# KirillHit/snn_for_object_detection

Measured on AMD Instinct MI355X. Metric: event-frames/sec (BxT) SODa-3M GEN1 304x240 fwd+bwd, higher is better.
Workload: dtype f32 (16-bit split products)

## Files before the change

### snn_for_object_detection_amd/csrc/conv_halo.hip

```cpp
#include <stdlib.h>
#include <type_traits>
#include "snn_common.h"

namespace {

constexpr int kThreads = 256;
constexpr int HBM_ = 128;
constexpr int HCELLS = 288;
constexpr int HPIECE = HCELLS * 64;
constexpr int NPASS = HCELLS / 32;
static_assert(NPASS == 9, "one halo staging pass per tap");

typedef __bf16 bf16x8 __attribute__((ext_vector_type(8)));
typedef __bf16 bf16x2 __attribute__((ext_vector_type(2)));
typedef _Float16 f16x8 __attribute__((ext_vector_type(8)));
typedef _Float16 f16x2 __attribute__((ext_vector_type(2)));
typedef float f32x2 __attribute__((ext_vector_type(2)));
typedef unsigned u32x2 __attribute__((ext_vector_type(2)));
typedef unsigned u32x4 __attribute__((ext_vector_type(4)));

constexpr float kF16WeightScale = 256.0f;
constexpr float kF16ActScale = 16.0f;
constexpr float kF16Unscale = 1.0f / (kF16WeightScale * kF16ActScale);

struct HaloGeom {
    int64_t ldx, ldy, ld_add, ld_add2;
    int N, H, W, Cin, Cout;
    int PW, PH;
    int G;
    int group_cells;
    int tiles_per_group, tiles, tiles_per_xcd, ntiles_n;
    unsigned magic_pw, magic_ph;
    int out_vec;
    double* bn_partial;
    int OH, OW;
    int tiles_x, tiles_img;
    float x_th;
};

__device__ __forceinline__ unsigned udiv_small(unsigned n, unsigned magic) { return __umulhi(n, magic); }

template <bool F16>
__device__ __forceinline__ void split4(const f32x4& v, u32x2& hi, u32x2& lo) {
#pragma unroll
    for (int e = 0; e < 4; e += 2) {
        if constexpr (F16) {
            const float a = v[e] * kF16ActScale, b = v[e + 1] * kF16ActScale;
            const f16x2 ph = __builtin_convertvector(f32x2{a, b}, f16x2);
            const f16x2 pl = __builtin_convertvector(f32x2{a - (float)ph[0], b - (float)ph[1]}, f16x2);
            hi[e >> 1] = __builtin_bit_cast(unsigned, ph);
            lo[e >> 1] = __builtin_bit_cast(unsigned, pl);
        } else {
            f32x2 rest = {v[e], v[e + 1]};
            const bf16x2 ph = __builtin_convertvector(rest, bf16x2);
            const unsigned bits = __builtin_bit_cast(unsigned, ph);
            rest[0] -= __builtin_bit_cast(float, bits << 16);
            rest[1] -= __builtin_bit_cast(float, bits & 0xffff0000u);
            const bf16x2 pl = __builtin_convertvector(rest, bf16x2);
            hi[e >> 1] = bits;
            lo[e >> 1] = __builtin_bit_cast(unsigned, pl);
        }
    }
}

__device__ __forceinline__ double partner8(double v) {
    const u32x2 u = __builtin_bit_cast(u32x2, v);
    const u32x2 o = {(unsigned)__builtin_amdgcn_update_dpp(0, (int)u[0], 0x128, 0xf, 0xf, false),
                     (unsigned)__builtin_amdgcn_update_dpp(0, (int)u[1], 0x128, 0xf, 0xf, false)};
    return __builtin_bit_cast(double, o);
}
__device__ __forceinline__ double partner16(double v) {
    const u32x2 u = __builtin_bit_cast(u32x2, v);
    const u32x2 o = {__builtin_amdgcn_permlane16_swap(u[0], u[0], false, false)[0],
                     __builtin_amdgcn_permlane16_swap(u[1], u[1], false, false)[0]};
    return __builtin_bit_cast(double, o);
}
__device__ __forceinline__ double partner32(double v) {
    const u32x2 u = __builtin_bit_cast(u32x2, v);
    const u32x2 o = {__builtin_amdgcn_permlane32_swap(u[0], u[0], false, false)[0],
                     __builtin_amdgcn_permlane32_swap(u[1], u[1], false, false)[0]};
    return __builtin_bit_cast(double, o);
}

__device__ __forceinline__ int cell_slot_off(int cell, int slot) { return cell * 64 + ((slot ^ ((cell >> 2) & 3)) << 4); }


constexpr int RTH = 4, RTW = 32, RPITCH = RTW + 2, RCELLS = (RTH + 2) * RPITCH;

template <int CO, bool F16, int ABL = 0, bool RECT = false, bool SBF = false, bool XSP = false>
__global__ __launch_bounds__(kThreads, 2) void k_conv_halo3(const float* __restrict__ x,
                                                           const unsigned char* __restrict__ wimg,
                                                           float* __restrict__ y, HaloGeom g,
                                                           const float* __restrict__ addend,
                                                           const float* __restrict__ addend2) {
    constexpr int WM = CO == 32 ? 4 : 2, WN = 4 / WM, TM = CO == 32 ? 1 : 2, TN = CO == 32 ? 1 : CO / 64;
    static_assert(CO == 32 || CO == 64 || CO == 128, "channel tile");
    constexpr int BTILE = (CO / 32) * 4096;
    constexpr int NDMA = (CO / 32) * 4 / 4;
    constexpr int ES = SBF ? 2 : 4;
    static_assert(!SBF || (!F16 && ABL == 0), "bf16 storage: bf16 MFMA, plain variant");
    static_assert(!XSP || (F16 && !SBF && ABL == 0), "spikes from potentials: the forward arithmetic, plain variant");
    constexpr int HC = RECT ? (RCELLS + 31) / 32 * 32 : HCELLS;
    constexpr int HP = HC * 64;
    constexpr int RED_BYTES = (F16 || SBF) ? 4 * (CO == 128 ? 64 : 32) * 16 : 0;
    __shared__ __attribute__((aligned(16))) unsigned char smem[2 * HP + 2 * BTILE + RED_BYTES];
    unsigned char* Aimg = smem;
    unsigned char* Bimg = smem + 2 * HP;

    const int tid = threadIdx.x, lane = tid & 63;
    const int wave = __builtin_amdgcn_readfirstlane(tid >> 6);
    const int wm = wave / WN, wn = wave % WN;
    const int r = lane & 31, h = lane >> 5;

    const int bq = blockIdx.x >> 3;
    const int tile = (blockIdx.x & 7) * g.tiles_per_xcd + bq / g.ntiles_n;
    if (tile >= g.tiles) return;
    const int n0c = (bq % g.ntiles_n) * CO;
    int grp, kt, c0 = 0, x0 = 0, y0 = 0, n0, nb;
    [[maybe_unused]] int ty = 0, tx = 0;
    if constexpr (RECT) {
        n0 = tile / g.tiles_img;
        const int rem = tile - n0 * g.tiles_img;
        ty = rem / g.tiles_x;
        tx = rem - ty * g.tiles_x;
        grp = n0 / g.G;
        kt = (n0 - grp * g.G) * g.tiles_img + rem;
        nb = n0;
    } else {
        grp = tile / g.tiles_per_group;
        kt = tile - grp * g.tiles_per_group;
        c0 = kt * HBM_;
        const int R0g = c0 / g.PW;
        x0 = c0 - R0g * g.PW;
        const int ng = R0g / g.PH;
        y0 = R0g - ng * g.PH;
        n0 = grp * g.G + ng;
        nb = n0 > 0 ? n0 - 1 : 0;
    }
    const int pitch = RECT ? RPITCH : g.PW;

    const int quad = tid & 7;
    const int64_t ipix = (int64_t)g.H * g.W;
    const int64_t xbytes = ((((int64_t)g.N - nb) * ipix - 1) * g.ldx + g.Cin) * ES;
    __amdgpu_buffer_rsrc_t rs_x = __builtin_amdgcn_make_buffer_rsrc(
        reinterpret_cast<char*>(const_cast<float*>(x)) + (int64_t)nb * ipix * g.ldx * ES, 0,
        xbytes > 0x7fffffffLL ? 0x7fffffff : (int)xbytes, 0x00020000);
    unsigned voff[NPASS];
    int awr[NPASS];
#pragma unroll
    for (int p = 0; p < NPASS; ++p) {
        const int cell = p * 32 + (tid >> 3);
        int xx, yy, n;
        bool ok;
        if constexpr (RECT) {
            const int rr = cell / RPITCH, cc = cell - rr * RPITCH;
            yy = ty * RTH - 1 + rr;
            xx = tx * RTW - 1 + cc;
            n = n0;
            ok = cell < RCELLS && yy >= 0 && yy < g.H && xx >= 0 && xx < g.W;
        } else {
            const unsigned u = (unsigned)(x0 + cell + g.PW - 1);
            const unsigned dR = udiv_small(u, g.magic_pw);
            xx = (int)(u - dR * g.PW);
            const unsigned v = (unsigned)(y0 + (int)dR + g.PH - 2);
            const unsigned dn = udiv_small(v, g.magic_ph);
            yy = (int)(v - dn * g.PH);
            n = n0 - 1 + (int)dn;
            ok = n >= 0 && n < g.N && xx < g.W && yy < g.H;
        }
        const int64_t pix = (int64_t)(n - nb) * ipix + (int64_t)yy * g.W + xx;
        voff[p] = ok ? (unsigned)((pix * g.ldx + quad * 4) * ES) : 0x80000000u;
        awr[p] = cell_slot_off(cell, quad >> 1) + (quad & 1) * 8;
    }

    int cellbase[TM];
#pragma unroll
    for (int i = 0; i < TM; ++i)
        cellbase[i] = RECT ? (wm * TM + i + 1) * RPITCH + 1 + r : g.PW + 1 + (wm * TM + i) * 32 + r;
    const int nchunks = g.Cin >> 5;
    const int co_tiles = g.Cout >> 5;
    const unsigned char* wsrc = wimg + (int64_t)(n0c >> 5) * 4096 + lane * 16;
    const unsigned lds_b = (unsigned)(size_t)(__attribute__((address_space(3))) unsigned char*)Bimg;
    auto dma_b = [&](int kk, int buf) {
        if constexpr (SBF)
            if (wave & 1) return;
        const int chunk = kk / 9, tap = kk - chunk * 9;
        const unsigned char* src = wsrc + ((int64_t)(tap * nchunks + chunk) * co_tiles) * 4096 + wave * 1024;
        const unsigned dst = lds_b + buf * BTILE + wave * 1024;
#pragma unroll
        for (int q = 0; q < NDMA; ++q) {
            unsigned keep;
            asm volatile("s_mov_b32 %0, m0\n\ts_mov_b32 m0, %2\n\ts_nop 0\n\tglobal_load_lds_dwordx4 %1, off\n\ts_mov_b32 m0, %0"
                         : "=&s"(keep)
                         : "v"(src + q * 4096), "s"(__builtin_amdgcn_readfirstlane(dst + q * 4096))
                         : "memory");
        }
    };

    using PReg = typename std::conditional<SBF, u32x2, f32x4>::type;
    PReg pf[NPASS];
    auto store_halo = [&]() {
#pragma unroll
        for (int p = 0; p < NPASS; ++p) {
            if constexpr (RECT)
                if (p * 32 >= HC) continue;
            if constexpr (SBF) {
                *reinterpret_cast<u32x2*>(Aimg + awr[p]) = pf[p];
            } else if constexpr (XSP) {
                const u32x2 hi = {(pf[p][0] > g.x_th ? 0x4C00u : 0u) | (pf[p][1] > g.x_th ? 0x4C000000u : 0u),
                                  (pf[p][2] > g.x_th ? 0x4C00u : 0u) | (pf[p][3] > g.x_th ? 0x4C000000u : 0u)};
                *reinterpret_cast<u32x2*>(Aimg + awr[p]) = hi;
            } else {
                u32x2 hi, lo;
                split4<F16>(pf[p], hi, lo);
                *reinterpret_cast<u32x2*>(Aimg + awr[p]) = hi;
                *reinterpret_cast<u32x2*>(Aimg + HP + awr[p]) = lo;
            }
        }
    };
    auto load_pass = [&](int off) -> PReg {
        if constexpr (SBF) return __builtin_bit_cast(u32x2, __builtin_amdgcn_raw_buffer_load_b64(rs_x, off, 0, 0));
        else return __builtin_bit_cast(f32x4, __builtin_amdgcn_raw_buffer_load_b128(rs_x, off, 0, 0));
    };

    f32x16 acc[TM][TN];
#pragma unroll
    for (int i = 0; i < TM; ++i)
#pragma unroll
        for (int j = 0; j < TN; ++j)
#pragma unroll
            for (int e = 0; e < 16; ++e) acc[i][j][e] = 0.f;

    auto kstep = [&](int tapoff, const unsigned char* Bb) {
#pragma unroll
        for (int ks = 0; ks < 2; ++ks) {
            bf16x8 ah[TM], al[TM], bh[TN], bl[TN];
#pragma unroll
            for (int i = 0; i < TM; ++i) {
                const int off = cell_slot_off(cellbase[i] + tapoff, 2 * ks + h);
                if constexpr (ABL & 16) {
                    if (i == 0 && ks == 0) ah[0] = *reinterpret_cast<const bf16x8*>(Aimg + off);
                    ah[i] = ah[0];
                    al[i] = ah[0];
                    continue;
                }
                ah[i] = *reinterpret_cast<const bf16x8*>(Aimg + off);
                if constexpr (!SBF && !XSP) al[i] = *reinterpret_cast<const bf16x8*>(Aimg + HP + off);
            }
#pragma unroll
            for (int j = 0; j < TN; ++j) {
                const int off = (wn * TN + j) * 4096 + ks * 2048 + lane * 16;
                bh[j] = *reinterpret_cast<const bf16x8*>(Bb + off);
                if constexpr (!SBF) bl[j] = *reinterpret_cast<const bf16x8*>(Bb + off + 1024);
            }
#pragma unroll
            for (int i = 0; i < TM; ++i)
#pragma unroll
                for (int j = 0; j < TN; ++j) {
                    if constexpr (SBF) {
                        acc[i][j] = __builtin_amdgcn_mfma_f32_32x32x16_bf16(ah[i], bh[j], acc[i][j], 0, 0, 0);
                    } else if constexpr (XSP) {
                        const f16x8 xah = __builtin_bit_cast(f16x8, ah[i]);
                        const f16x8 xbh = __builtin_bit_cast(f16x8, bh[j]), xbl = __builtin_bit_cast(f16x8, bl[j]);
                        acc[i][j] = __builtin_amdgcn_mfma_f32_32x32x16_f16(xah, xbl, acc[i][j], 0, 0, 0);
                        acc[i][j] = __builtin_amdgcn_mfma_f32_32x32x16_f16(xah, xbh, acc[i][j], 0, 0, 0);
                    } else if constexpr (F16) {
                        const f16x8 xah = __builtin_bit_cast(f16x8, ah[i]), xal = __builtin_bit_cast(f16x8, al[i]);
                        const f16x8 xbh = __builtin_bit_cast(f16x8, bh[j]), xbl = __builtin_bit_cast(f16x8, bl[j]);
                        acc[i][j] = __builtin_amdgcn_mfma_f32_32x32x16_f16(xal, xbh, acc[i][j], 0, 0, 0);
                        acc[i][j] = __builtin_amdgcn_mfma_f32_32x32x16_f16(xah, xbl, acc[i][j], 0, 0, 0);
                        acc[i][j] = __builtin_amdgcn_mfma_f32_32x32x16_f16(xah, xbh, acc[i][j], 0, 0, 0);
                    } else {
                        acc[i][j] = __builtin_amdgcn_mfma_f32_32x32x16_bf16(al[i], bh[j], acc[i][j], 0, 0, 0);
                        acc[i][j] = __builtin_amdgcn_mfma_f32_32x32x16_bf16(ah[i], bl[j], acc[i][j], 0, 0, 0);
                        acc[i][j] = __builtin_amdgcn_mfma_f32_32x32x16_bf16(ah[i], bh[j], acc[i][j], 0, 0, 0);
                    }
                }
        }
    };

    dma_b(0, 0);
#pragma unroll
    for (int p = 0; p < NPASS; ++p) pf[p] = load_pass((int)voff[p]);
    store_halo();
    asm volatile("s_waitcnt vmcnt(0) lgkmcnt(0)\n\ts_barrier" ::: "memory");

    const int nk = nchunks * 9;
#pragma unroll 1
    for (int chunk = 0; chunk < nchunks; ++chunk) {
        const bool more = chunk + 1 < nchunks;
        const int cbytes = (chunk + 1) * 32 * ES;
#pragma unroll
        for (int tap = 0; tap < 9; ++tap) {
            const int kk = chunk * 9 + tap;
            const int cur = kk & 1;
            if constexpr (!(ABL & 1))
                if (kk + 1 < nk) dma_b(kk + 1, cur ^ 1);
            __builtin_amdgcn_sched_barrier(0);
            if constexpr (!(ABL & 4)) {
                if (more) pf[tap] = load_pass((int)(voff[tap] + (unsigned)cbytes));
            }
            __builtin_amdgcn_sched_barrier(0);
            const int kh = tap / 3, kw = tap - 3 * kh;
            kstep((kh - 1) * pitch + (kw - 1), Bimg + cur * BTILE);
            if constexpr (ABL & 2) asm volatile("" ::: "memory");
            else if constexpr (ABL & 4) asm volatile("s_waitcnt vmcnt(0) lgkmcnt(0)\n\ts_barrier" ::: "memory");
            else asm volatile("s_waitcnt vmcnt(0) lgkmcnt(0)\n\ts_barrier" ::: "memory");
        }
        if (more) {
            store_halo();
            asm volatile("s_waitcnt lgkmcnt(0)\n\ts_barrier" ::: "memory");
        }
    }

    constexpr int EW = TN * 32 + 4;
    constexpr int LPR = TN * 8;
    constexpr int RPP = 64 / LPR;
    float* stage = reinterpret_cast<float*>(smem) + wave * 32 * EW;
    const bool ovec = g.out_vec != 0;
    const int lrow = lane / LPR, c4 = (lane % LPR) * 4;
    const int nch = n0c + wn * TN * 32 + c4;
    const int cells_left = g.group_cells - c0;
    double ssum[4] = {0.0, 0.0, 0.0, 0.0}, qsum[4] = {0.0, 0.0, 0.0, 0.0};
    const bool stats = (F16 || SBF) && g.bn_partial != nullptr;
    auto cell_pixel = [&](int m, int64_t& pix) -> bool {
        int xx, yy, n;
        bool ok;
        if constexpr (RECT) {
            yy = ty * RTH + (m >> 5);
            xx = tx * RTW + (m & 31);
            n = n0;
            ok = yy < g.H && xx < g.W && nch < g.Cout;
        } else {
            const unsigned u = (unsigned)(x0 + m);
            const unsigned dR = udiv_small(u, g.magic_pw);
            xx = (int)(u - dR * g.PW);
            const unsigned v = (unsigned)(y0 + (int)dR);
            const unsigned dn = udiv_small(v, g.magic_ph);
            yy = (int)(v - dn * g.PH);
            n = n0 + (int)dn;
            ok = m < cells_left && xx < g.W && yy < g.H && n < g.N && nch < g.Cout;
        }
        pix = ((int64_t)n * g.H + yy) * g.W + xx;
        return ok;
    };
    typedef SnnStore<SBF> St;
    constexpr int NPS = 32 / RPP;
    const bool prefetch_add = ovec && (addend != nullptr || addend2 != nullptr) && !(ABL & 8);
#pragma unroll
    for (int i = 0; i < TM; ++i) {
        f32x4 pa1[NPS], pa2[NPS];
        int64_t ppix[NPS];
        unsigned okmask = 0;
        if (prefetch_add) {
#pragma unroll
            for (int pass = 0; pass < NPS; ++pass) {
                const bool ok = cell_pixel((wm * TM + i) * 32 + pass * RPP + lrow, ppix[pass]);
                okmask |= ok ? 1u << pass : 0u;
                const int64_t pc = ok ? ppix[pass] : 0;
                const int nc = ok ? nch : 0;
                const f32x4 zero = {0.f, 0.f, 0.f, 0.f};
                pa1[pass] = addend ? St::ld4_last(addend, pc * g.ld_add + nc) : zero;
                pa2[pass] = addend2 ? St::ld4_last(addend2, pc * g.ld_add2 + nc) : zero;
            }
        }
#pragma unroll
        for (int j = 0; j < TN; ++j)
#pragma unroll
            for (int e = 0; e < 16; ++e)
                stage[((e & 3) + 8 * (e >> 2) + 4 * h) * EW + j * 32 + r] = F16 ? acc[i][j][e] * kF16Unscale : acc[i][j][e];
        asm volatile("s_waitcnt lgkmcnt(0)" ::: "memory");
        if (prefetch_add) {
#pragma unroll
            for (int pass = 0; pass < NPS; ++pass) {
                f32x4 val = *reinterpret_cast<const f32x4*>(&stage[(pass * RPP + lrow) * EW + c4]);
                if (addend) val += pa1[pass];
                if (addend2) val += pa2[pass];
                if ((okmask >> pass) & 1u) St::st4(y, ppix[pass] * g.ldy + nch, val);
            }
            asm volatile("s_waitcnt lgkmcnt(0)" ::: "memory");
            continue;
        }
#pragma unroll
        for (int pass = 0; pass < NPS; ++pass) {
            const int row = pass * RPP + lrow;
            int64_t pix;
            const bool ok = cell_pixel((wm * TM + i) * 32 + row, pix);
            f32x4 val = *reinterpret_cast<const f32x4*>(&stage[row * EW + c4]);
            if (!ok) continue;
            if constexpr (ABL & 8) {
                asm volatile("" :: "v"(val[0]), "v"(val[1]), "v"(val[2]), "v"(val[3]));
                continue;
            }
            if (ovec) {
                if (addend) val += St::ld4_last(addend, pix * g.ld_add + nch);
                if (addend2) val += St::ld4_last(addend2, pix * g.ld_add2 + nch);
                St::st4(y, pix * g.ldy + nch, val);
            } else {
#pragma unroll
                for (int q = 0; q < 4; ++q) {
                    float o = val[q];
                    if (addend) o += St::ld1(addend, pix * g.ld_add + nch + q);
                    if (addend2) o += St::ld1(addend2, pix * g.ld_add2 + nch + q);
                    St::st1(y, pix * g.ldy + nch + q, o);
                }
            }
            if (stats) {
#pragma unroll
                for (int q = 0; q < 4; ++q) {
                    const double d = (double)val[q];
                    ssum[q] += d;
                    qsum[q] = fma(d, d, qsum[q]);
                }
            }
        }
        asm volatile("s_waitcnt lgkmcnt(0)" ::: "memory");
    }
    if (stats) {
#pragma unroll
        for (int q = 0; q < 4; ++q) {
            if constexpr (LPR <= 8) {
                ssum[q] += partner8(ssum[q]);
                qsum[q] += partner8(qsum[q]);
            }
            ssum[q] += partner16(ssum[q]);
            qsum[q] += partner16(qsum[q]);
            ssum[q] += partner32(ssum[q]);
            qsum[q] += partner32(qsum[q]);
        }
        double* red = reinterpret_cast<double*>(smem + 2 * HP + 2 * BTILE);
        if (lane >= 48 && lane < 48 + LPR) {
#pragma unroll
            for (int q = 0; q < 4; ++q) {
                red[((wave * LPR + lane - 48) * 4 + q) * 2 + 0] = ssum[q];
                red[((wave * LPR + lane - 48) * 4 + q) * 2 + 1] = qsum[q];
            }
        }
        __syncthreads();
        if (tid < CO) {
            const int wn_ = tid / (TN * 32), cc = tid % (TN * 32);
            double s = 0.0, q2 = 0.0;
#pragma unroll
            for (int wm_ = 0; wm_ < WM; ++wm_) {
                const double* src = red + (((wm_ * WN + wn_) * LPR * 4) + cc) * 2;
                s += src[0];
                q2 += src[1];
            }
            if (n0c + tid < g.Cout) {
                double* dstp = g.bn_partial + snn_bn_partial_index(grp, kt, n0c + tid, g.tiles_per_group, g.Cout);
                dstp[0] = s;
                dstp[1] = q2;
            }
        }
    }
}

constexpr int SPITCH = RTW + 1, SCELLS = (RTH + 1) * SPITCH;
template <bool SBF = false, bool RECT = false>
__global__ __launch_bounds__(kThreads, 2) void k_conv_s2dgrad3(const float* __restrict__ x,
                                                              const unsigned char* __restrict__ wimg,
                                                              float* __restrict__ y,
                                                              HaloGeom g, const float* __restrict__ addend,
                                                              const float* __restrict__ addend2) {
    constexpr int CO = 64, TN = 2;
    constexpr int ES = SBF ? 2 : 4;
    constexpr int BTILE = (CO / 32) * 4096;
    constexpr int NDMA = (CO / 32) * 4 / 4;
    __shared__ __attribute__((aligned(16))) unsigned char smem[2 * HPIECE + 2 * BTILE];
    unsigned char* Aimg = smem;
    unsigned char* Bimg = smem + 2 * HPIECE;

    const int tid = threadIdx.x, lane = tid & 63;
    const int wave = __builtin_amdgcn_readfirstlane(tid >> 6);
    const int r = lane & 31, h = lane >> 5;

    const int bq = blockIdx.x >> 3;
    const int tile = (blockIdx.x & 7) * g.tiles_per_xcd + bq / g.ntiles_n;
    if (tile >= g.tiles) return;
    const int n0c = (bq % g.ntiles_n) * CO;
    int c0 = 0, x0 = 0, y0 = 0, n0;
    [[maybe_unused]] int ty = 0, tx = 0;
    if constexpr (RECT) {
        n0 = tile / g.tiles_img;
        const int rem = tile - n0 * g.tiles_img;
        ty = rem / g.tiles_x;
        tx = rem - ty * g.tiles_x;
    } else {
        c0 = tile * HBM_;
        const int R0g = c0 / g.PW;
        x0 = c0 - R0g * g.PW;
        n0 = R0g / g.PH;
        y0 = R0g - n0 * g.PH;
    }
    const int nb = n0;
    const int pitch = RECT ? SPITCH : g.PW;

    const int quad = tid & 7;
    const int64_t ipix = (int64_t)g.H * g.W;
    const int64_t xbytes = ((((int64_t)g.N - nb) * ipix - 1) * g.ldx + g.Cin) * ES;
    __amdgpu_buffer_rsrc_t rs_x = __builtin_amdgcn_make_buffer_rsrc(
        reinterpret_cast<char*>(const_cast<float*>(x)) + (int64_t)nb * ipix * g.ldx * ES, 0,
        xbytes > 0x7fffffffLL ? 0x7fffffff : (int)xbytes, 0x00020000);
    unsigned voff[NPASS];
    int awr[NPASS];
#pragma unroll
    for (int p = 0; p < NPASS; ++p) {
        const int cell = p * 32 + (tid >> 3);
        int xx, yy, n;
        bool ok;
        if constexpr (RECT) {
            const int rr = cell / SPITCH, cc = cell - rr * SPITCH;
            yy = ty * RTH + rr;
            xx = tx * RTW + cc;
            n = n0;
            ok = cell < SCELLS && xx < g.W && yy < g.H;
        } else {
            const unsigned u = (unsigned)(x0 + cell);
            const unsigned dR = udiv_small(u, g.magic_pw);
            xx = (int)(u - dR * g.PW);
            const unsigned v = (unsigned)(y0 + (int)dR);
            const unsigned dn = udiv_small(v, g.magic_ph);
            yy = (int)(v - dn * g.PH);
            n = n0 + (int)dn;
            ok = n < g.N && xx < g.W && yy < g.H;
        }
        const int64_t pix = (int64_t)(n - nb) * ipix + (int64_t)yy * g.W + xx;
        voff[p] = ok ? (unsigned)((pix * g.ldx + quad * 4) * ES) : 0x80000000u;
        awr[p] = cell_slot_off(cell, quad >> 1) + (quad & 1) * 8;
    }
    const int cellbase = RECT ? wave * SPITCH + r : wave * 32 + r;
    const int nchunks = g.Cin >> 5;
    const int co_tiles = g.Cout >> 5;
    const unsigned char* wsrc = wimg + (int64_t)(n0c >> 5) * 4096 + lane * 16;
    const unsigned lds_b = (unsigned)(size_t)(__attribute__((address_space(3))) unsigned char*)Bimg;
    auto dma_b = [&](int kk, int buf) {
        if constexpr (SBF)
            if (wave & 1) return;
        const int chunk = kk / 9, tap = kk - chunk * 9;
        const unsigned char* src = wsrc + ((int64_t)((8 - tap) * nchunks + chunk) * co_tiles) * 4096 + wave * 1024;
        const unsigned dst = lds_b + buf * BTILE + wave * 1024;
#pragma unroll
        for (int q = 0; q < NDMA; ++q) {
            unsigned keep;
            asm volatile("s_mov_b32 %0, m0\n\ts_mov_b32 m0, %2\n\ts_nop 0\n\tglobal_load_lds_dwordx4 %1, off\n\ts_mov_b32 m0, %0"
                         : "=&s"(keep)
                         : "v"(src + q * 4096), "s"(__builtin_amdgcn_readfirstlane(dst + q * 4096))
                         : "memory");
        }
    };
    using PReg = typename std::conditional<SBF, u32x2, f32x4>::type;
    PReg pf[NPASS];
    auto store_halo = [&]() {
#pragma unroll
        for (int p = 0; p < NPASS; ++p) {
            if constexpr (SBF) {
                *reinterpret_cast<u32x2*>(Aimg + awr[p]) = pf[p];
            } else {
                u32x2 hi, lo;
                split4<false>(pf[p], hi, lo);
                *reinterpret_cast<u32x2*>(Aimg + awr[p]) = hi;
                *reinterpret_cast<u32x2*>(Aimg + HPIECE + awr[p]) = lo;
            }
        }
    };
    auto load_pass = [&](int off) -> PReg {
        if constexpr (SBF) return __builtin_bit_cast(u32x2, __builtin_amdgcn_raw_buffer_load_b64(rs_x, off, 0, 0));
        else return __builtin_bit_cast(f32x4, __builtin_amdgcn_raw_buffer_load_b128(rs_x, off, 0, 0));
    };
    f32x16 acc[4][TN];
#pragma unroll
    for (int c = 0; c < 4; ++c)
#pragma unroll
        for (int j = 0; j < TN; ++j)
#pragma unroll
            for (int e = 0; e < 16; ++e) acc[c][j][e] = 0.f;

    auto kstep = [&](int tapoff, const unsigned char* Bb, f32x16 (&a)[TN]) {
#pragma unroll
        for (int ks = 0; ks < 2; ++ks) {
            const int off = cell_slot_off(cellbase + tapoff, 2 * ks + h);
            const bf16x8 ah = *reinterpret_cast<const bf16x8*>(Aimg + off);
            bf16x8 al = ah;
            if constexpr (!SBF) al = *reinterpret_cast<const bf16x8*>(Aimg + HPIECE + off);
#pragma unroll
            for (int j = 0; j < TN; ++j) {
                const int boff = j * 4096 + ks * 2048 + lane * 16;
                const bf16x8 bh = *reinterpret_cast<const bf16x8*>(Bb + boff);
                if constexpr (!SBF) {
                    const bf16x8 bl = *reinterpret_cast<const bf16x8*>(Bb + boff + 1024);
                    a[j] = __builtin_amdgcn_mfma_f32_32x32x16_bf16(al, bh, a[j], 0, 0, 0);
                    a[j] = __builtin_amdgcn_mfma_f32_32x32x16_bf16(ah, bl, a[j], 0, 0, 0);
                }
                a[j] = __builtin_amdgcn_mfma_f32_32x32x16_bf16(ah, bh, a[j], 0, 0, 0);
            }
        }
    };

    dma_b(0, 0);
#pragma unroll
    for (int p = 0; p < NPASS; ++p) pf[p] = load_pass((int)voff[p]);
    store_halo();
    asm volatile("s_waitcnt vmcnt(0) lgkmcnt(0)\n\ts_barrier" ::: "memory");

    const int nk = nchunks * 9;
#pragma unroll 1
    for (int chunk = 0; chunk < nchunks; ++chunk) {
        const bool more = chunk + 1 < nchunks;
        const int cbytes = (chunk + 1) * 32 * ES;
#pragma unroll
        for (int tap = 0; tap < 9; ++tap) {
            const int kk = chunk * 9 + tap;
            const int cur = kk & 1;
            if (kk + 1 < nk) dma_b(kk + 1, cur ^ 1);
            __builtin_amdgcn_sched_barrier(0);
            if (more) pf[tap] = load_pass((int)(voff[tap] + (unsigned)cbytes));
            __builtin_amdgcn_sched_barrier(0);
            const int kh = tap / 3, kw = tap - 3 * kh;
            const int ph = kh == 1 ? 0 : 1, pw = kw == 1 ? 0 : 1;
            const int dh = kh == 0 ? 1 : 0, dw = kw == 0 ? 1 : 0;
            kstep(dh * pitch + dw, Bimg + cur * BTILE, acc[2 * ph + pw]);
            asm volatile("s_waitcnt vmcnt(0) lgkmcnt(0)\n\ts_barrier" ::: "memory");
        }
        if (more) {
            store_halo();
            asm volatile("s_waitcnt lgkmcnt(0)\n\ts_barrier" ::: "memory");
        }
    }

    constexpr int EW = TN * 32 + 4, LPR = TN * 8, RPP = 64 / LPR;
    float* stage = reinterpret_cast<float*>(smem) + wave * 32 * EW;
    const bool ovec = g.out_vec != 0;
    const int lrow = lane / LPR, c4 = (lane % LPR) * 4;
    const int nch = n0c + c4;
    const int cells_left = g.group_cells - c0;
#pragma unroll
    for (int cls = 0; cls < 4; ++cls) {
        const int ph = cls >> 1, pw = cls & 1;
#pragma unroll
        for (int j = 0; j < TN; ++j)
#pragma unroll
            for (int e = 0; e < 16; ++e)
                stage[((e & 3) + 8 * (e >> 2) + 4 * h) * EW + j * 32 + r] = acc[cls][j][e];
        asm volatile("s_waitcnt lgkmcnt(0)" ::: "memory");
#pragma unroll
        for (int pass = 0; pass < 32 / RPP; ++pass) {
            const int row = pass * RPP + lrow;
            const int m = wave * 32 + row;
            int aa, bb, n;
            bool inside;
            if constexpr (RECT) {
                aa = ty * RTH + wave;
                bb = tx * RTW + row;
                n = n0;
                inside = true;
            } else {
                const unsigned u = (unsigned)(x0 + m);
                const unsigned dR = udiv_small(u, g.magic_pw);
                bb = (int)(u - dR * g.PW);
                const unsigned v = (unsigned)(y0 + (int)dR);
                const unsigned dn = udiv_small(v, g.magic_ph);
                aa = (int)(v - dn * g.PH);
                n = n0 + (int)dn;
                inside = m < cells_left && n < g.N;
            }
            const int hi = 2 * aa + ph, wi = 2 * bb + pw;
            const bool ok = inside && bb < g.W && aa < g.H && hi < g.OH && wi < g.OW && nch < g.Cout;
            f32x4 val = *reinterpret_cast<const f32x4*>(&stage[row * EW + c4]);
            if (!ok) continue;
            const int64_t pix = ((int64_t)n * g.OH + hi) * g.OW + wi;
            typedef SnnStore<SBF> St;
            if (ovec) {
                if (addend) val += St::ld4_last(addend, pix * g.ld_add + nch);
                if (addend2) val += St::ld4_last(addend2, pix * g.ld_add2 + nch);
                St::st4(y, pix * g.ldy + nch, val);
            } else {
#pragma unroll
                for (int q = 0; q < 4; ++q) {
                    float o = val[q];
                    if (addend) o += St::ld1(addend, pix * g.ld_add + nch + q);
                    if (addend2) o += St::ld1(addend2, pix * g.ld_add2 + nch + q);
                    St::st1(y, pix * g.ldy + nch + q, o);
                }
            }
        }
        asm volatile("s_waitcnt lgkmcnt(0)" ::: "memory");
    }
}

template <bool F16>
__global__ void k_weight_frag_image(const float* __restrict__ flat_src, unsigned char* __restrict__ flat_dst,
                                    const int64_t* __restrict__ table, int flip) {
    const int64_t* row = table + (int64_t)blockIdx.y * 4;
    const float* src = flat_src + row[0];
    unsigned char* dst = flat_dst + row[1];
    const int O = (int)row[2], I = (int)row[3];
    const int ot_n = O >> 5, ic_n = I >> 5;
    const int64_t total = (int64_t)9 * ic_n * ot_n * 2 * 64;
    for (int64_t idx = (int64_t)blockIdx.x * blockDim.x + threadIdx.x; idx < total; idx += (int64_t)gridDim.x * blockDim.x) {
        const int lane = (int)(idx & 63);
        const int ks = (int)((idx >> 6) & 1);
        int64_t rest = idx >> 7;
        const int ot = (int)(rest % ot_n); rest /= ot_n;
        const int ic = (int)(rest % ic_n);
        const int tap = (int)(rest / ic_n);
        const int r = lane & 31, h = lane >> 5;
        const int st = flip ? 8 - tap : tap;
        const float* p = src + ((int64_t)(ot * 32 + r) * 9 + st) * I + ic * 32 + ks * 16 + h * 8;
        const f32x4 v0 = *reinterpret_cast<const f32x4*>(p), v1 = *reinterpret_cast<const f32x4*>(p + 4);
        u32x4 hi, lo;
#pragma unroll
        for (int e = 0; e < 8; e += 2) {
            const float a0 = e < 4 ? v0[e] : v1[e - 4], a1 = e < 4 ? v0[e + 1] : v1[e - 3];
            if (F16) {
                const float a = a0 * kF16WeightScale, b = a1 * kF16WeightScale;
                const f16x2 ph = __builtin_convertvector(f32x2{a, b}, f16x2);
                const f16x2 pl = __builtin_convertvector(f32x2{a - (float)ph[0], b - (float)ph[1]}, f16x2);
                hi[e >> 1] = __builtin_bit_cast(unsigned, ph);
                lo[e >> 1] = __builtin_bit_cast(unsigned, pl);
            } else {
                f32x2 rr = {a0, a1};
                const bf16x2 ph = __builtin_convertvector(rr, bf16x2);
                const unsigned bits = __builtin_bit_cast(unsigned, ph);
                rr[0] -= __builtin_bit_cast(float, bits << 16);
                rr[1] -= __builtin_bit_cast(float, bits & 0xffff0000u);
                const bf16x2 pl = __builtin_convertvector(rr, bf16x2);
                hi[e >> 1] = bits;
                lo[e >> 1] = __builtin_bit_cast(unsigned, pl);
            }
        }
        unsigned char* o = dst + ((((int64_t)(tap * ic_n + ic) * ot_n + ot) * 2 + ks) * 2) * 1024 + lane * 16;
        *reinterpret_cast<u32x4*>(o) = hi;
        *reinterpret_cast<u32x4*>(o + 1024) = lo;
    }
}

static int halo_mode(int64_t N, int H, int W, int Cin, int Cout) {
    if (N <= 0 || H <= 0 || W <= 0) return 0;
    if (Cin % 32 != 0 || Cin < 32 || (Cout % 64 != 0 && Cout != 32)) return 0;
    if (W + 1 <= 79) {
        if (N * (int64_t)(H + 1) * (W + 1) >= 0x7fffffffLL) return 0;
        return 1;
    }
    const int64_t tiles = N * snn_ceil_div(H, RTH) * snn_ceil_div(W, RTW);
    return tiles < 0x7fffffffLL ? 2 : 0;
}
static bool halo_shape_ok(int64_t N, int H, int W, int Cin, int Cout) { return halo_mode(N, H, W, Cin, Cout) != 0; }

static bool s2dgrad_rect(int Wo) { return 128 + (Wo + 1) + 2 > HCELLS; }
static bool s2dgrad_shape_ok(int64_t N, int H, int W, int Cin, int Ho, int Wo, int Cout) {
    if (N <= 0 || H <= 0 || W <= 0) return false;
    if (Ho != (H - 1) / 2 + 1 || Wo != (W - 1) / 2 + 1) return false;
    if (Cout % 32 != 0 || Cout < 32 || Cin % 64 != 0) return false;
    if (s2dgrad_rect(Wo)) return N * snn_ceil_div(Ho, RTH) * snn_ceil_div(Wo, RTW) < 0x7fffffffLL;
    if (N * (int64_t)(Ho + 1) * (Wo + 1) >= 0x7fffffffLL) return false;
    return true;
}

struct HaloPlan {
    int mode;
    int co_tile, ntiles_n;
    int G;
    int tiles_x, tiles_img;
    int group_cells;
    int tiles_per_group, tiles, tiles_per_xcd, grid;
};
static void plan_grid(HaloPlan& p) {
    if (p.tiles * (int64_t)p.ntiles_n + 8 >= 0x7fffffffLL) {
        p.mode = 0;
        return;
    }
    p.tiles_per_xcd = (int)snn_ceil_div(p.tiles, 8);
    const int64_t grid = (int64_t)p.tiles_per_xcd * 8 * p.ntiles_n;
    if (grid > 0x7fffffffLL) p.mode = 0;
    p.grid = (int)grid;
}
static HaloPlan halo_plan(int64_t N, int H, int W, int Cin, int Cout, int G) {
    HaloPlan p = {};
    p.mode = halo_mode(N, H, W, Cin, Cout);
    if (p.mode == 0 || G <= 0 || N % G != 0) return HaloPlan{};
    p.G = G;
    p.co_tile = Cout % 128 == 0 ? 128 : (Cout % 64 == 0 ? 64 : 32);
    p.ntiles_n = Cout / p.co_tile;
    p.tiles_x = (int)snn_ceil_div(W, RTW);
    p.tiles_img = p.tiles_x * (int)snn_ceil_div(H, RTH);
    int64_t tiles;
    if (p.mode == 2) {
        p.tiles_per_group = G * p.tiles_img;
        tiles = N * (int64_t)p.tiles_img;
    } else {
        const int64_t group_cells = (int64_t)G * (H + 1) * (W + 1);
        p.group_cells = (int)group_cells;
        p.tiles_per_group = (int)snn_ceil_div(group_cells, HBM_);
        tiles = (N / G) * p.tiles_per_group;
    }
    if (tiles >= 0x7fffffffLL) return HaloPlan{};
    p.tiles = (int)tiles;
    plan_grid(p);
    return p;
}
static HaloPlan s2dgrad_plan(int64_t N, int H, int W, int Cin, int Ho, int Wo, int Cout) {
    HaloPlan p = {};
    if (!s2dgrad_shape_ok(N, H, W, Cin, Ho, Wo, Cout)) return p;
    p.mode = s2dgrad_rect(Wo) ? 2 : 1;
    p.G = (int)N;
    p.co_tile = 64;
    p.ntiles_n = Cin / 64;
    p.tiles_x = (int)snn_ceil_div(Wo, RTW);
    p.tiles_img = p.tiles_x * (int)snn_ceil_div(Ho, RTH);
    if (p.mode == 2) {
        p.tiles_per_group = p.tiles_img;
        p.tiles = (int)(N * p.tiles_img);
    } else {
        const int64_t cells = N * (int64_t)(Ho + 1) * (Wo + 1);
        p.group_cells = (int)cells;
        p.tiles_per_group = (int)snn_ceil_div(cells, HBM_);
        p.tiles = p.tiles_per_group;
    }
    plan_grid(p);
    return p;
}
static int plan_out(const HaloPlan& p, int* out) {
    const int v[7] = {p.mode, p.co_tile, p.tiles, p.tiles_per_group, p.tiles_per_xcd, p.ntiles_n, p.grid};
    for (int i = 0; i < 7; ++i) out[i] = v[i];
    return p.mode == 0 ? 1 : 0;
}

static HaloGeom halo_geom(const HaloPlan& hp, int64_t N, int H, int W, int Cin, int64_t ld_in, int OH, int OW, int Cout,
                          const void* out, int64_t ld_out, const void* addend, int64_t ld_add, const void* addend2,
                          int64_t ld_add2, bool bf16, double* bn_partial, float x_th) {
    HaloGeom g = {};
    g.ldx = ld_in; g.ldy = ld_out; g.ld_add = ld_add; g.ld_add2 = ld_add2;
    g.N = (int)N; g.H = H; g.W = W; g.Cin = Cin; g.Cout = Cout;
    g.OH = OH; g.OW = OW;
    g.PW = W + 1; g.PH = H + 1;
    g.G = hp.G;
    g.tiles_x = hp.tiles_x;
    g.tiles_img = hp.tiles_img;
    g.group_cells = hp.group_cells;
    g.tiles_per_group = hp.tiles_per_group;
    g.tiles = hp.tiles;
    g.ntiles_n = hp.ntiles_n;
    g.tiles_per_xcd = hp.tiles_per_xcd;
    g.magic_pw = magic_u32(g.PW); g.magic_ph = magic_u32(g.PH);
    g.out_vec = multiples(4, {ld_out, addend ? ld_add : 0, addend2 ? ld_add2 : 0}) && aligned(bf16 ? 8 : 16, {out, addend, addend2});
    g.bn_partial = bn_partial;
    g.x_th = x_th;
    return g;
}
}

extern "C" int snn_conv3x3_s2_dgrad_supported(int64_t N, int H, int W, int Cin, int Ho, int Wo, int Cout) {
    return s2dgrad_shape_ok(N, H, W, Cin, Ho, Wo, Cout) ? 1 : 0;
}

extern "C" int snn_conv3x3_s2_dgrad(const float* dy, int64_t lddy, const void* wt_image, float* dx, int64_t lddx, int64_t N,
                                    int H, int W, int Cin, int Ho, int Wo, int Cout, const float* addend, int64_t ld_addend,
                                    const float* addend2, int64_t ld_addend2, int precision, void* stream) {
    SNN_REQUIRE(dy && wt_image && dx, "snn_conv3x3_s2_dgrad: null pointer");
    SNN_REQUIRE(precision == SNN_PREC_BF16X3 || precision == SNN_PREC_BF16S,
                "snn_conv3x3_s2_dgrad: precision must be SNN_PREC_BF16X3 or SNN_PREC_BF16S (got %d)", precision);
    const bool sbf = precision == SNN_PREC_BF16S;
    SNN_REQUIRE(s2dgrad_shape_ok(N, H, W, Cin, Ho, Wo, Cout),
                "snn_conv3x3_s2_dgrad: shape not covered (N %lld, %dx%d -> %dx%d, %d -> %d channels; ask "
                "snn_conv3x3_s2_dgrad_supported)", (long long)N, H, W, Ho, Wo, Cin, Cout);
    SNN_REQUIRE(lddy >= Cout && lddx >= Cin && lddy % 4 == 0, "snn_conv3x3_s2_dgrad: bad pixel strides (%lld, %lld)",
                (long long)lddy, (long long)lddx);
    SNN_REQUIRE(aligned(sbf ? 8 : 16, {dy}) && aligned(16, {wt_image}),
                "snn_conv3x3_s2_dgrad: dy (16 bytes; 8 for bf16) and the weight image (16) must be aligned");
    SNN_REQUIRE(!addend || ld_addend >= Cin, "snn_conv3x3_s2_dgrad: addend pixel stride smaller than channel count");
    SNN_REQUIRE(!addend2 || ld_addend2 >= Cin, "snn_conv3x3_s2_dgrad: addend2 pixel stride smaller than channel count");
    const HaloPlan hp = s2dgrad_plan(N, H, W, Cin, Ho, Wo, Cout);
    SNN_REQUIRE(hp.mode != 0, "snn_conv3x3_s2_dgrad: grid too large");
    const bool rect = hp.mode == 2;
    if (rect)
        SNN_REQUIRE((int64_t)Ho * Wo * lddy * 4 < 0x7fffffffLL, "snn_conv3x3_s2_dgrad: a dy image must span less than 2 GiB");
    else
        SNN_REQUIRE((int64_t)4 * Ho * Wo * lddy * 4 < 0x7fffffffLL, "snn_conv3x3_s2_dgrad: four dy images must span less than 2 GiB");
    const HaloGeom g = halo_geom(hp, N, Ho, Wo, Cout, lddy, H, W, Cin, dx, lddx, addend, ld_addend, addend2, ld_addend2, sbf,
                                 nullptr, 0.0f);
    dispatch(
        [&](auto SBF, auto RECT) {
            hipLaunchKernelGGL((k_conv_s2dgrad3<SBF(), RECT()>), dim3((unsigned)hp.grid), dim3(kThreads), 0, (hipStream_t)stream,
                               dy, static_cast<const unsigned char*>(wt_image), dx, g, addend, addend2);
            return true;
        },
        Flag{sbf}, Flag{rect});
    SNN_CHECK_LAUNCH("snn_conv3x3_s2_dgrad");
    return 0;
}

extern "C" int snn_conv3x3_s2_dgrad_plan(int64_t N, int H, int W, int Cin, int Ho, int Wo, int Cout, int* out) {
    if (!out) return 1;
    return plan_out(s2dgrad_plan(N, H, W, Cin, Ho, Wo, Cout), out);
}

extern "C" int snn_conv3x3_halo_supported(int64_t N, int H, int W, int Cin, int Cout) {
    return halo_shape_ok(N, H, W, Cin, Cout) ? 1 : 0;
}

extern "C" int snn_conv3x3_halo_plan(int64_t N, int H, int W, int Cin, int Cout, int frames_per_step, int* out) {
    if (!out) return 1;
    return plan_out(halo_plan(N, H, W, Cin, Cout, frames_per_step > 0 ? frames_per_step : (int)N), out);
}

extern "C" int64_t snn_conv3x3_halo_bn_chunks(int frames_per_step, int H, int W) {
    if (W + 1 <= 79) return snn_ceil_div((int64_t)frames_per_step * (H + 1) * (W + 1), HBM_);
    return (int64_t)frames_per_step * snn_ceil_div(H, RTH) * snn_ceil_div(W, RTW);
}

extern "C" size_t snn_weight_frag_image_bytes(int O, int I) { return (size_t)9 * O * I * 4; }

extern "C" int snn_weight_frag_image_batched(const float* flat_src, void* flat_dst, const int64_t* table, int n,
                                             int max_groups, int flip, int precision, void* stream) {
    SNN_REQUIRE(flat_src && flat_dst && table && n > 0 && max_groups > 0, "snn_weight_frag_image_batched: bad arguments");
    SNN_REQUIRE(precision == SNN_PREC_FP16X3 || precision == SNN_PREC_BF16X3,
                "snn_weight_frag_image: precision must be SNN_PREC_FP16X3 (forward) or SNN_PREC_BF16X3 (data gradient)");
    SNN_REQUIRE(aligned(16, {flat_src, flat_dst}), "snn_weight_frag_image: buffers must be 16-byte aligned");
    int64_t bx = snn_ceil_div(max_groups, kThreads);
    if (bx > 64) bx = 64;
    dim3 grid((unsigned)bx, (unsigned)n);
    dispatch(
        [&](auto F16) {
            hipLaunchKernelGGL(k_weight_frag_image<F16()>, grid, dim3(kThreads), 0, (hipStream_t)stream, flat_src,
                               static_cast<unsigned char*>(flat_dst), table, flip);
            return true;
        },
        Flag{precision == SNN_PREC_FP16X3});
    SNN_CHECK_LAUNCH("snn_weight_frag_image_batched");
    return 0;
}

static int conv3x3_halo_impl(const float* x, int64_t ldx, const void* w_image, float* y, int64_t ldy, int64_t N, int H,
                             int W, int Cin, int Cout, const float* addend, int64_t ld_addend, const float* addend2,
                             int64_t ld_addend2, double* bn_partial, int frames_per_step, int* bn_layout,
                             int precision, void* stream, bool xsp, float x_th) {
    SNN_REQUIRE(x && w_image && y, "snn_conv3x3_halo: null pointer");
    SNN_REQUIRE(precision == SNN_PREC_FP16X3 || precision == SNN_PREC_BF16X3 || precision == SNN_PREC_BF16S,
                "snn_conv3x3_halo: precision must be SNN_PREC_FP16X3, SNN_PREC_BF16X3 or SNN_PREC_BF16S (got %d)", precision);
    const bool sbf = precision == SNN_PREC_BF16S;
    SNN_REQUIRE(halo_shape_ok(N, H, W, Cin, Cout),
                "snn_conv3x3_halo: shape not covered (N %lld, %dx%d, %d -> %d channels; ask snn_conv3x3_halo_supported)",
                (long long)N, H, W, Cin, Cout);
    SNN_REQUIRE(ldx >= Cin && ldy >= Cout && ldx % 4 == 0, "snn_conv3x3_halo: bad pixel strides (%lld, %lld)",
                (long long)ldx, (long long)ldy);
    SNN_REQUIRE(aligned(sbf ? 8 : 16, {x}) && aligned(16, {w_image}),
                "snn_conv3x3_halo: x (16 bytes; 8 for bf16) and the weight image (16) must be aligned");
    SNN_REQUIRE(!addend || ld_addend >= Cout, "snn_conv3x3_halo: addend pixel stride smaller than channel count");
    SNN_REQUIRE(!addend2 || ld_addend2 >= Cout, "snn_conv3x3_halo: addend2 pixel stride smaller than channel count");
    SNN_REQUIRE(!bn_partial || ((precision == SNN_PREC_FP16X3 || sbf) && bn_layout && frames_per_step > 0 &&
                                N % frames_per_step == 0 && !addend && !addend2),
                "snn_conv3x3_halo: statistics need the forward arithmetic, bn_layout, no addend and a frames_per_step "
                "that divides N (%lld frames, %d per step)", (long long)N, frames_per_step);
    SNN_REQUIRE((int64_t)4 * H * W * ldx * 4 < 0x7fffffffLL, "snn_conv3x3_halo: four images must span less than 2 GiB");
    if (bn_layout) bn_layout[0] = bn_layout[1] = 0;
    const HaloPlan hp = halo_plan(N, H, W, Cin, Cout, bn_partial ? frames_per_step : (int)N);
    SNN_REQUIRE(hp.mode != 0, "snn_conv3x3_halo: grid too large");
    const bool rect = hp.mode == 2;
    if (rect) SNN_REQUIRE((int64_t)H * W * ldx * 4 < 0x7fffffffLL, "snn_conv3x3_halo: an image must span less than 2 GiB");
    const HaloGeom g = halo_geom(hp, N, H, W, Cin, ldx, H, W, Cout, y, ldy, addend, ld_addend, addend2, ld_addend2, sbf,
                                 bn_partial, x_th);
    if (bn_partial) bn_layout[0] = g.tiles_per_group;
    const dim3 grid((unsigned)hp.grid);
    const unsigned char* wi = static_cast<const unsigned char*>(w_image);
#ifdef SNN_TUNING
    if (const char* e = snn_tuning_env("SNN_HALO_ABL")) {
        const bool launched = dispatch(
            [&](auto ABL, auto CO) {
                hipLaunchKernelGGL((k_conv_halo3<CO(), true, ABL()>), grid, dim3(kThreads), 0, (hipStream_t)stream, x, wi, y, g,
                                   addend, addend2);
                return true;
            },
            OneOf<1, 2, 4, 8, 16, 3, 7, 15, 31>{atoi(e)}, OneOf<64, 128>{hp.co_tile == 128 ? 128 : 64});
        if (launched) {
            SNN_CHECK_LAUNCH("snn_conv3x3_halo");
            return 0;
        }
    }
#endif
    enum { kPieces = 0, kBf16Storage = 1, kSpikes = 2 };
    const bool f16 = precision == SNN_PREC_FP16X3;
    dispatch(
        [&](auto CO, auto RECT, auto OPERAND, auto F16) {
            if constexpr (OPERAND() == kPieces || F16() == (OPERAND() == kSpikes)) {
                hipLaunchKernelGGL((k_conv_halo3<CO(), F16(), 0, RECT(), OPERAND() == kBf16Storage, OPERAND() == kSpikes>), grid,
                                   dim3(kThreads), 0, (hipStream_t)stream, x, wi, y, g, addend, addend2);
            }
            return true;
        },
        OneOf<32, 64, 128>{hp.co_tile}, Flag{rect}, OneOf<0, 1, 2>{xsp ? kSpikes : (sbf ? kBf16Storage : kPieces)}, Flag{f16});
    SNN_CHECK_LAUNCH(xsp ? "snn_conv3x3_halo_spikes" : "snn_conv3x3_halo");
    return 0;
}

extern "C" int snn_conv3x3_halo(const float* x, int64_t ldx, const void* w_image, float* y, int64_t ldy, int64_t N, int H,
                                int W, int Cin, int Cout, const float* addend, int64_t ld_addend, const float* addend2,
                                int64_t ld_addend2, double* bn_partial, int frames_per_step, int* bn_layout,
                                int precision, void* stream) {
    return conv3x3_halo_impl(x, ldx, w_image, y, ldy, N, H, W, Cin, Cout, addend, ld_addend, addend2, ld_addend2, bn_partial,
                             frames_per_step, bn_layout, precision, stream, false, 0.0f);
}

extern "C" int snn_conv3x3_halo_spikes(const float* vdec, int64_t ld, float v_th, const void* w_image, float* y, int64_t ldy,
                                       int64_t N, int H, int W, int Cin, int Cout, double* bn_partial, int frames_per_step,
                                       int* bn_layout, void* stream) {
    SNN_REQUIRE(v_th >= 0.0f, "snn_conv3x3_halo_spikes: a negative threshold would turn padding into spikes");
    return conv3x3_halo_impl(vdec, ld, w_image, y, ldy, N, H, W, Cin, Cout, nullptr, 0, nullptr, 0, bn_partial,
                             frames_per_step, bn_layout, SNN_PREC_FP16X3, stream, true, v_th);
}
```

Measured before the change: 7401.

## Group three taps per pipeline stage and shrink halo LDS in s2 dgrad

The stride-2 dgrad kernel now stages weights for three taps per double-buffered step, so there are three barriers per input chunk instead of nine. The halo buffer is sized per variant: narrow strip tiles use 224 cells, and cells beyond the needed extent are masked. The LDS freed by the smaller halo pays for the larger weight buffers while keeping two blocks per CU. A WIDE variant keeps the old one-tap, 288-cell layout for wide images, which adds one more template dimension to the dispatch.

```diff
diff --git a/snn_for_object_detection_amd/csrc/conv_halo.hip b/snn_for_object_detection_amd/csrc/conv_halo.hip
--- a/snn_for_object_detection_amd/csrc/conv_halo.hip
+++ b/snn_for_object_detection_amd/csrc/conv_halo.hip
@@ -7,7 +7,6 @@
 constexpr int kThreads = 256;
 constexpr int HBM_ = 128;
 constexpr int HCELLS = 288;
-constexpr int HPIECE = HCELLS * 64;
 constexpr int NPASS = HCELLS / 32;
 static_assert(NPASS == 9, "one halo staging pass per tap");
 
@@ -456,19 +455,29 @@
 }
 
 constexpr int SPITCH = RTW + 1, SCELLS = (RTH + 1) * SPITCH;
-template <bool SBF = false, bool RECT = false>
+constexpr int SHC_NARROW = 224, SHC_RECT = (SCELLS + 31) / 32 * 32;
+template <bool SBF = false, bool RECT = false, bool WIDE = false>
 __global__ __launch_bounds__(kThreads, 2) void k_conv_s2dgrad3(const float* __restrict__ x,
                                                               const unsigned char* __restrict__ wimg,
                                                               float* __restrict__ y,
                                                               HaloGeom g, const float* __restrict__ addend,
                                                               const float* __restrict__ addend2) {
+    static_assert(!WIDE || (!SBF && !RECT), "one-tap stages: fp32 strip tiles only");
     constexpr int CO = 64, TN = 2;
     constexpr int ES = SBF ? 2 : 4;
     constexpr int BTILE = (CO / 32) * 4096;
     constexpr int NDMA = (CO / 32) * 4 / 4;
-    __shared__ __attribute__((aligned(16))) unsigned char smem[2 * HPIECE + 2 * BTILE];
+    constexpr int TS = WIDE ? 1 : 3;
+    constexpr int NST = 9 / TS;
+    constexpr int HC = RECT ? SHC_RECT : (SBF || WIDE) ? HCELLS : SHC_NARROW;
+    constexpr int HP = HC * 64;
+    constexpr int NP = HC / 32;
+    constexpr int PPS = (NP + NST - 1) / NST;
+    __shared__ __attribute__((aligned(16))) unsigned char smem[(SBF ? 1 : 2) * HP + 2 * TS * BTILE];
+    static_assert(2 * sizeof(smem) <= 160 * 1024, "two blocks per CU");
+    static_assert(sizeof(smem) >= 4 * 32 * (TN * 32 + 4) * 4, "the epilogue stages 32 x 64 floats per wave");
     unsigned char* Aimg = smem;
-    unsigned char* Bimg = smem + 2 * HPIECE;
+    unsigned char* Bimg = smem + (SBF ? 1 : 2) * HP;
 
     const int tid = threadIdx.x, lane = tid & 63;
     const int wave = __builtin_amdgcn_readfirstlane(tid >> 6);
@@ -501,10 +510,10 @@
     __amdgpu_buffer_rsrc_t rs_x = __builtin_amdgcn_make_buffer_rsrc(
         reinterpret_cast<char*>(const_cast<float*>(x)) + (int64_t)nb * ipix * g.ldx * ES, 0,
         xbytes > 0x7fffffffLL ? 0x7fffffff : (int)xbytes, 0x00020000);
-    unsigned voff[NPASS];
-    int awr[NPASS];
-#pragma unroll
-    for (int p = 0; p < NPASS; ++p) {
+    unsigned voff[NP];
+    int awr[NP];
+#pragma unroll
+    for (int p = 0; p < NP; ++p) {
         const int cell = p * 32 + (tid >> 3);
         int xx, yy, n;
         bool ok;
@@ -522,7 +531,7 @@
             const unsigned dn = udiv_small(v, g.magic_ph);
             yy = (int)(v - dn * g.PH);
             n = n0 + (int)dn;
-            ok = n < g.N && xx < g.W && yy < g.H;
+            ok = n < g.N && xx < g.W && yy < g.H && cell <= HBM_ + g.PW;
         }
         const int64_t pix = (int64_t)(n - nb) * ipix + (int64_t)yy * g.W + xx;
         voff[p] = ok ? (unsigned)((pix * g.ldx + quad * 4) * ES) : 0x80000000u;
@@ -533,33 +542,36 @@
     const int co_tiles = g.Cout >> 5;
     const unsigned char* wsrc = wimg + (int64_t)(n0c >> 5) * 4096 + lane * 16;
     const unsigned lds_b = (unsigned)(size_t)(__attribute__((address_space(3))) unsigned char*)Bimg;
-    auto dma_b = [&](int kk, int buf) {
+    auto dma_b = [&](int ss, int buf) {
         if constexpr (SBF)
             if (wave & 1) return;
-        const int chunk = kk / 9, tap = kk - chunk * 9;
-        const unsigned char* src = wsrc + ((int64_t)((8 - tap) * nchunks + chunk) * co_tiles) * 4096 + wave * 1024;
-        const unsigned dst = lds_b + buf * BTILE + wave * 1024;
-#pragma unroll
-        for (int q = 0; q < NDMA; ++q) {
-            unsigned keep;
-            asm volatile("s_mov_b32 %0, m0\n\ts_mov_b32 m0, %2\n\ts_nop 0\n\tglobal_load_lds_dwordx4 %1, off\n\ts_mov_b32 m0, %0"
-                         : "=&s"(keep)
-                         : "v"(src + q * 4096), "s"(__builtin_amdgcn_readfirstlane(dst + q * 4096))
-                         : "memory");
+        const int chunk = ss / NST, tap0 = (ss - chunk * NST) * TS;
+#pragma unroll
+        for (int t = 0; t < TS; ++t) {
+            const unsigned char* src = wsrc + ((int64_t)((8 - tap0 - t) * nchunks + chunk) * co_tiles) * 4096 + wave * 1024;
+            const unsigned dst = lds_b + (buf * TS + t) * BTILE + wave * 1024;
+#pragma unroll
+            for (int q = 0; q < NDMA; ++q) {
+                unsigned keep;
+                asm volatile("s_mov_b32 %0, m0\n\ts_mov_b32 m0, %2\n\ts_nop 0\n\tglobal_load_lds_dwordx4 %1, off\n\ts_mov_b32 m0, %0"
+                             : "=&s"(keep)
+                             : "v"(src + q * 4096), "s"(__builtin_amdgcn_readfirstlane(dst + q * 4096))
+                             : "memory");
+            }
         }
     };
     using PReg = typename std::conditional<SBF, u32x2, f32x4>::type;
-    PReg pf[NPASS];
+    PReg pf[NP];
     auto store_halo = [&]() {
 #pragma unroll
-        for (int p = 0; p < NPASS; ++p) {
+        for (int p = 0; p < NP; ++p) {
             if constexpr (SBF) {
                 *reinterpret_cast<u32x2*>(Aimg + awr[p]) = pf[p];
             } else {
                 u32x2 hi, lo;
                 split4<false>(pf[p], hi, lo);
                 *reinterpret_cast<u32x2*>(Aimg + awr[p]) = hi;
-                *reinterpret_cast<u32x2*>(Aimg + HPIECE + awr[p]) = lo;
+                *reinterpret_cast<u32x2*>(Aimg + HP + awr[p]) = lo;
             }
         }
     };
@@ -581,7 +593,7 @@
             const int off = cell_slot_off(cellbase + tapoff, 2 * ks + h);
             const bf16x8 ah = *reinterpret_cast<const bf16x8*>(Aimg + off);
             bf16x8 al = ah;
-            if constexpr (!SBF) al = *reinterpret_cast<const bf16x8*>(Aimg + HPIECE + off);
+            if constexpr (!SBF) al = *reinterpret_cast<const bf16x8*>(Aimg + HP + off);
 #pragma unroll
             for (int j = 0; j < TN; ++j) {
                 const int boff = j * 4096 + ks * 2048 + lane * 16;
@@ -598,27 +610,34 @@
 
     dma_b(0, 0);
 #pragma unroll
-    for (int p = 0; p < NPASS; ++p) pf[p] = load_pass((int)voff[p]);
+    for (int p = 0; p < NP; ++p) pf[p] = load_pass((int)voff[p]);
     store_halo();
     asm volatile("s_waitcnt vmcnt(0) lgkmcnt(0)\n\ts_barrier" ::: "memory");
 
-    const int nk = nchunks * 9;
+    const int nss = nchunks * NST;
 #pragma unroll 1
     for (int chunk = 0; chunk < nchunks; ++chunk) {
         const bool more = chunk + 1 < nchunks;
         const int cbytes = (chunk + 1) * 32 * ES;
 #pragma unroll
-        for (int tap = 0; tap < 9; ++tap) {
-            const int kk = chunk * 9 + tap;
-            const int cur = kk & 1;
-            if (kk + 1 < nk) dma_b(kk + 1, cur ^ 1);
+        for (int st = 0; st < NST; ++st) {
+            const int ss = chunk * NST + st;
+            const int cur = ss & 1;
+            if (ss + 1 < nss) dma_b(ss + 1, cur ^ 1);
             __builtin_amdgcn_sched_barrier(0);
-            if (more) pf[tap] = load_pass((int)(voff[tap] + (unsigned)cbytes));
+            if (more) {
+#pragma unroll
+                for (int p = st * PPS; p < (st + 1) * PPS && p < NP; ++p) pf[p] = load_pass((int)(voff[p] + (unsigned)cbytes));
+            }
             __builtin_amdgcn_sched_barrier(0);
-            const int kh = tap / 3, kw = tap - 3 * kh;
-            const int ph = kh == 1 ? 0 : 1, pw = kw == 1 ? 0 : 1;
-            const int dh = kh == 0 ? 1 : 0, dw = kw == 0 ? 1 : 0;
-            kstep(dh * pitch + dw, Bimg + cur * BTILE, acc[2 * ph + pw]);
+#pragma unroll
+            for (int t = 0; t < TS; ++t) {
+                const int tap = st * TS + t;
+                const int kh = tap / 3, kw = tap - 3 * kh;
+                const int ph = kh == 1 ? 0 : 1, pw = kw == 1 ? 0 : 1;
+                const int dh = kh == 0 ? 1 : 0, dw = kw == 0 ? 1 : 0;
+                kstep(dh * pitch + dw, Bimg + (cur * TS + t) * BTILE, acc[2 * ph + pw]);
+            }
             asm volatile("s_waitcnt vmcnt(0) lgkmcnt(0)\n\ts_barrier" ::: "memory");
         }
         if (more) {
@@ -878,13 +897,15 @@
         SNN_REQUIRE((int64_t)4 * Ho * Wo * lddy * 4 < 0x7fffffffLL, "snn_conv3x3_s2_dgrad: four dy images must span less than 2 GiB");
     const HaloGeom g = halo_geom(hp, N, Ho, Wo, Cout, lddy, H, W, Cin, dx, lddx, addend, ld_addend, addend2, ld_addend2, sbf,
                                  nullptr, 0.0f);
+    const bool wide = !sbf && !rect && HBM_ + (Wo + 1) + 2 > SHC_NARROW;
     dispatch(
-        [&](auto SBF, auto RECT) {
-            hipLaunchKernelGGL((k_conv_s2dgrad3<SBF(), RECT()>), dim3((unsigned)hp.grid), dim3(kThreads), 0, (hipStream_t)stream,
-                               dy, static_cast<const unsigned char*>(wt_image), dx, g, addend, addend2);
+        [&](auto SBF, auto RECT, auto WIDE) {
+            if constexpr (!WIDE() || (!SBF() && !RECT()))
+                hipLaunchKernelGGL((k_conv_s2dgrad3<SBF(), RECT(), WIDE()>), dim3((unsigned)hp.grid), dim3(kThreads), 0,
+                                   (hipStream_t)stream, dy, static_cast<const unsigned char*>(wt_image), dx, g, addend, addend2);
             return true;
         },
-        Flag{sbf}, Flag{rect});
+        Flag{sbf}, Flag{rect}, Flag{wide});
     SNN_CHECK_LAUNCH("snn_conv3x3_s2_dgrad");
     return 0;
 }
```

Result: no change. 7420, median of 5 (+0.3%).
